# anibali/dsnt-pose2d

Measured on AMD Instinct MI355X. Metric: images/sec (train step, 256x256, 16 joints), higher is better.
Workload: dtype f32; 1 GPU; hg2 + DSNT + JS reg, 256x256 -> 64x64x16, batch 32 per GPU, RMSprop lr 2.5e-4, train step fwd+loss+bwd+optim; global_batch=32, parallelism=dp1, launches_fwd=210

## Files before the change

### dsnt-pose2d_amd/csrc/api.cpp

```cpp
#include "common.h"
#include <string.h>

static thread_local char g_err[512] = "";

int dsnt_set_error(int code, const char* fmt, ...) {
    va_list ap;
    va_start(ap, fmt);
    vsnprintf(g_err, sizeof(g_err), fmt, ap);
    va_end(ap);
    return code;
}

int dsnt_device_id(void) {
    int d = 0;
    if (hipGetDevice(&d) != hipSuccess || d < 0) d = 0;
    return d < DSNT_MAX_DEVICES ? d : DSNT_MAX_DEVICES - 1;
}

int dsnt_device_cus(void) {
    static std::atomic<int> cus[DSNT_MAX_DEVICES];
    const int d = dsnt_device_id();
    int c = cus[d].load(std::memory_order_acquire);
    if (!c) {
        hipDeviceProp_t prop;
        int dev = 0;
        c = (hipGetDevice(&dev) == hipSuccess && hipGetDeviceProperties(&prop, dev) == hipSuccess && prop.multiProcessorCount > 0)
                ? prop.multiProcessorCount : 256;
        cus[d].store(c, std::memory_order_release);
    }
    return c;
}

extern "C" int dsnt_version(void) { return 132; }
extern "C" const char* dsnt_last_error(void) { return g_err; }

#include <vector>
#include <new>

struct dsnt_list {
    struct Entry {
        int kind;
        int lane, src, dst;
        mutable hipEvent_t ev;
        std::function<void(hipStream_t)> fn;
    };
    std::vector<Entry> entries;
    std::vector<size_t> seg_start;
    dsnt_list() { seg_start.push_back(0); }
};

static thread_local dsnt_list* g_rec = nullptr;

dsnt_list* dsnt_recording(void) { return g_rec; }

void dsnt_record_launch(dsnt_list* l, int lane, std::function<void(hipStream_t)>&& fn) {
    dsnt_list::Entry e;
    e.kind = 0; e.lane = lane; e.src = e.dst = 0; e.ev = nullptr; e.fn = std::move(fn);
    l->entries.push_back(std::move(e));
}

extern "C" dsnt_list* dsnt_list_create(void) { return new (std::nothrow) dsnt_list(); }

extern "C" void dsnt_list_destroy(dsnt_list* l) {
    if (!l) return;
    if (g_rec == l) g_rec = nullptr;
    for (auto& e : l->entries)
// ... 60 lines not shown
```

### dsnt-pose2d_amd/csrc/bn.hip

```cpp
#include "common.h"
#include <string.h>
#include "bn_pro.h"
#include "ew_bodies.h"

template <int MODE>
__global__ __launch_bounds__(256) void tile_reduce_kernel(
    const float* __restrict__ a, const float* __restrict__ x, const float* __restrict__ scale,
    const float* __restrict__ shift, const float* __restrict__ mean,
    const float* __restrict__ invstd, int relu, float* __restrict__ partial, long M, int C, int cgs,
    const float* __restrict__ ymask = nullptr, float* __restrict__ dz_out = nullptr) {
    __shared__ float red[256 * 8];
    const int tid = threadIdx.x;
    const int C4 = C >> 2;
    const int rpar = 256 / cgs;
    const int cg_l = tid % cgs, rl = tid / cgs;
    const bool active = rl < rpar;
    const long row0 = (long)blockIdx.x * TILE_ROWS;
    const long row1 = row0 + TILE_ROWS < M ? row0 + TILE_ROWS : M;
    for (int cg0 = blockIdx.y * cgs; cg0 < C4; cg0 += cgs * gridDim.y) {
        const int cg = cg0 + cg_l;
        float4 s1 = make_float4(0.f, 0.f, 0.f, 0.f), s2 = s1;
        if (active && cg < C4) {
            float4 sc, sh, mu, is;
            if (MODE == 1) {
// ... 452 lines not shown

static int bn_bwd_pro_fill(BnBwdProP& q, const char* who, const float* partial, int ntiles, float* dgamma, float* dbeta,
                           int accumulate_params, float* coef, int64_t M, int C) {
    DSNT_REQUIRE(partial && ntiles > 0 && coef && C <= 256 && (long)ntiles * C <= 16384, DSNT_ERR_ARG,
                 "%s: needs partial sums of at most 256 channels / 128 KB and a coef buffer", who);
    q.partial = partial; q.tiles = ntiles; q.C = C; q.invM = 1.0 / (double)M;
    q.dgamma = dgamma; q.dbeta = dbeta; q.accumulate = accumulate_params; q.coef = coef;
    return DSNT_OK;
}

extern "C" int dsnt_bn_act_bwd_apply_pro(const float* da, const float* x, const float* scale, const float* shift,
                                         const float* mean, const float* invstd, const float* partial, int ntiles,
                                         float* dgamma, float* dbeta, int accumulate_params, float* coef, int relu,
                                         float* dx, int accumulate, int64_t M, int C, float* amax, void* stream) {
    BnBwdProP q;
    if (int e = bn_bwd_pro_fill(q, "dsnt_bn_act_bwd_apply_pro", partial, ntiles, dgamma, dbeta, accumulate_params, coef, M, C)) return e;
    return bn_act_bwd_apply_impl(da, x, scale, shift, mean, invstd, coef, relu, dx, accumulate, M, C, amax, stream, &q, nullptr);
}
extern "C" int dsnt_bn_act_bwd_apply_base(const float* da, const float* x, const float* scale, const float* shift,
                                          const float* mean, const float* invstd, const float* coef, int relu,
                                          const float* base, float* dx, int64_t M, int C, float* amax, void* stream) {
    DSNT_REQUIRE(base && base != dx, DSNT_ERR_ARG, "dsnt_bn_act_bwd_apply_base: `base` must be a second tensor");
    return bn_act_bwd_apply_impl(da, x, scale, shift, mean, invstd, coef, relu, dx, 1, M, C, amax, stream, nullptr, base);
}
extern "C" int dsnt_bn_act_bwd_apply_pro_base(const float* da, const float* x, const float* scale, const float* shift,
                                              const float* mean, const float* invstd, const float* partial, int ntiles,
                                              float* dgamma, float* dbeta, int accumulate_params, float* coef, int relu,
                                              const float* base, float* dx, int64_t M, int C, float* amax, void* stream) {
    DSNT_REQUIRE(base && base != dx, DSNT_ERR_ARG, "dsnt_bn_act_bwd_apply_pro_base: `base` must be a second tensor");
    BnBwdProP q;
    if (int e = bn_bwd_pro_fill(q, "dsnt_bn_act_bwd_apply_pro_base", partial, ntiles, dgamma, dbeta, accumulate_params, coef, M, C)) return e;
    return bn_act_bwd_apply_impl(da, x, scale, shift, mean, invstd, coef, relu, dx, 1, M, C, amax, stream, &q, base);
}
```

### dsnt-pose2d_amd/dsnt/_lib.py

```python
import ctypes as C
import os

import torch

_HERE = os.path.dirname(os.path.abspath(__file__))
LIB_PATH = os.environ.get('DSNT_HIP_LIB') or os.path.join(os.path.dirname(_HERE), 'csrc', 'libdsnt_hip.so')

P = C.c_void_p
I = C.c_int
L = C.c_int64
F = C.c_float
D = C.c_double


class ConvGeom(C.Structure):
    _fields_ = [(n, C.c_int) for n in
                ('N', 'H', 'W', 'Cin', 'Ho', 'Wo', 'Cout', 'R', 'S', 'stride', 'pad', 'dil')]


GP = C.POINTER(ConvGeom)


class BnBwdEpilogue(C.Structure):
    _fields_ = [('x', C.c_void_p), ('scale', C.c_void_p), ('shift', C.c_void_p), ('mean', C.c_void_p),
# ... 64 lines not shown
    'dsnt_conv_pack_dgrad': [P, P, I, I, I, I, P],
    'dsnt_conv_pack_dgrad_all': [P, I, P, P, P, L, P],
    'dsnt_conv_fwd_bf16x6': [P, P, L, P, P, P, P, I, P, P, P, GP, P],
    'dsnt_split_bf16x3': [P, P, L, P],
    'dsnt_conv_fwd_f16x3_ex': [P, P, L, P, P, P, P, P, P, I, P, P, P, GP, BP, TP, P],
    'dsnt_conv_fwd_f16x3_stream': [P, P, L, P, P, P, P, P, P, I, P, P, P, GP, BP, TP, P],
    'dsnt_amax': [P, L, P, P],
    'dsnt_split_f16x2': [P, P, L, L, P, P],
    'dsnt_f16_prep_weights': [P, I, I, P],
    'dsnt_f16_prep_bn_bounds': [P, I, P],
    'dsnt_conv_wgrad': [P, P, P, I, P, P, P, P, I, GP, P],
    'dsnt_conv_wgrad_bf16x6': [P, P, P, I, P, P, P, P, I, GP, P],
    'dsnt_conv_wgrad_f16x3': [P, P, P, I, P, P, P, P, I, P, P, GP, P],
    'dsnt_conv1x1_fwd_f16x3': [P, P, L, P, P, P, P, P, P, I, P, P, GP, TP, P],
    'dsnt_conv1x1_bwd_f16x3': [BP, P, AP, P, L, P, P, P, P, P, P, P, I, GP, P],
    'dsnt_conv1x1_fwd_ds_f16x3': [P, P, P, P, L, P, P, P, P, P, P, P, P, P, I, P, GP, GP, TP, P],
    'dsnt_conv_dgrad_f16x3_stream_apply': [P, AP, P, P, L, P, P, P, P, I, GP, BP, TP, P],
    'dsnt_wgrad_reduce_all': [P, I, I, P],
    'dsnt_conv_wgrad_group': [P, I, I, P],
    'dsnt_bn_stats': [P, P, L, I, P],
    'dsnt_bn_finalize': [P, I, L, I, P, P, P, P, F, F, I, P, P, P, P, P],
    'dsnt_bn_act_fwd': [P, P, P, I, P, L, I, P],
    'dsnt_bn_act_bwd_reduce': [P, P, P, P, P, P, I, P, L, I, P],
    'dsnt_bn_bwd_finalize': [P, I, L, I, P, P, I, P, P],
    'dsnt_bn_bwd_finalize_bound': [P, I, L, I, P, P, I, P, P, P, P, P],
    'dsnt_bn_eval_prep': [P, I, P],
    'dsnt_bn_act_bwd_apply': [P, P, P, P, P, P, P, I, P, I, L, I, P],
    'dsnt_bn_act_bwd_apply_amax': [P, P, P, P, P, P, P, I, P, I, L, I, P, P],
    'dsnt_bn_act_bwd_apply_pro': [P, P, P, P, P, P, P, I, P, P, I, P, I, P, I, L, I, P, P],
    'dsnt_stem4_fwd_f16x3': [P, P, L, P, P, P, P, P, GP, TP, P],
    'dsnt_bn_add_act_bwd_reduce': [P, P, P, P, P, I, P, P, L, I, P],
    'dsnt_bn_act_bwd_apply_base': [P, P, P, P, P, P, P, I, P, P, L, I, P, P],
    'dsnt_bn_act_bwd_apply_pro_base': [P, P, P, P, P, P, P, I, P, P, I, P, I, P, P, L, I, P, P],
    'dsnt_conv_fwd_pro': [P, P, P, P, PP, I, P, P, P, GP, TP, P],
    'dsnt_fill_zero': [P, L, P],
    'dsnt_axpy_amax': [P, P, F, I, L, P, P],
    'dsnt_maxpool2_bwd_amax': [P, P, P, I, I, I, I, I, P, P],
    'dsnt_maxpool2_bwd_add': [P, P, P, I, P, I, I, I, I, P, P],
    'dsnt_upsample2_bwd_amax': [P, P, I, I, I, I, I, P, P],
    'dsnt_maxpool2_fwd': [P, P, P, I, I, I, I, P],
    'dsnt_maxpool2_bwd': [P, P, P, I, I, I, I, I, P],
    'dsnt_maxpool2_fwd_stats': [P, P, P, P, I, I, I, I, TP, P],
    'dsnt_upsample2_add_fwd_stats': [P, P, P, P, I, I, I, I, TP, P],
    'dsnt_bn_act_fwd_stats': [P, P, P, I, P, P, L, I, TP, P],
    'dsnt_s2d_input': [P, P, I, I, I, I, TP, P],
    'dsnt_s2d_weights': [P, P, I, I, P],
    'dsnt_s2d_weights_prep': [P, P, P, P, P, I, P],
    'dsnt_maxpool3s2_fwd': [P, P, P, I, I, I, I, P],
    'dsnt_maxpool3s2_bwd': [P, P, P, I, I, I, I, I, P],
    'dsnt_bn_add_act_fwd': [P, P, P, P, I, P, L, I, P],
    'dsnt_relu_bwd': [P, P, P, L, P],
    'dsnt_zero_insert': [P, P, I, I, I, I, I, I, I, P],
    'dsnt_conv_dgrad_strided': [P, P, P, P, P, GP, BP, TP, P],
    'dsnt_upsample2_add_fwd': [P, P, P, I, I, I, I, P],
    'dsnt_upsample2_bwd': [P, P, I, I, I, I, I, P],
    'dsnt_axpy': [P, P, F, I, L, P],
    'dsnt_nchw_to_nhwc': [P, P, I, I, I, I, P],
    'dsnt_nhwc_to_nchw': [P, P, I, I, I, I, P],
    'dsnt_rmsprop_step': [P, P, P, L, F, F, F, F, F, P],
    'dsnt_sgd_step': [P, P, P, L, F, F, F, F, I, P],
    'dsnt_rmsprop_step_guarded': [P, P, P, L, F, F, F, F, F, P, P],
    'dsnt_sgd_step_guarded': [P, P, P, L, F, F, F, F, I, P, P],
    'dsnt_nonfinite_flag': [P, L, P, I, P],
    'dsnt_pckh': [P, P, P, P, P, P, F, P, P, I, I, P],
    'dsnt_pckh_hist': [P, P, P, P, P, P, P, I, P, P, I, I, P],
    'dsnt_error_field': [P, P, P, P, P, P, F, P, I, P, P, I, I, P],
# ... 113 lines not shown
```

### dsnt-pose2d_amd/dsnt/engine.py

```python
import os

import torch

from . import _lib, convop
from ._lib import ConvGeom, BnTail
from .bounds import Bounds
from .launchlist import Lanes, LaunchList
from .wgrad_queue import WgradQueue

BN_EPS = 1e-5
BN_MOMENTUM = 0.1


class Act:
    __slots__ = ('buf', 'N', 'H', 'W', 'C', '_grad', 'stats', 'name', 'grad_amax', 'amax_tail', 'fold_ok',
                 'pending_apply', 'uses', 'gives_away', 'is_branch', 'grad_shared', 'pending_add', 'base', 'base_amax')

    def __init__(self, buf, name=''):
        self.buf = buf
        self.N, self.H, self.W, self.C = buf.shape
        self._grad = None
        self.base, self.base_amax = None, None
        self.stats = None
        self.amax_tail = None
# ... 29 lines not shown
class ConvParams:
    __slots__ = ('w', 'b', 'gw', 'gb', 'Cout', 'R', 'S', 'Cin', 'stride', 'pad', 'dil', 'wq', 'wq_stride', 'wq16', 'wb',
                 'post_reduce')

    def __init__(self, w, b, gw, gb, stride=1, pad=0, dil=1):
        self.w, self.b, self.gw, self.gb = w, b, gw, gb
        self.wq, self.wq_stride = None, 0
        self.wq16, self.wb = None, None
        self.post_reduce = None
        self.Cout, self.R, self.S, self.Cin = w.shape
        self.stride, self.pad, self.dil = stride, pad, dil


class BnParams:
    __slots__ = ('gamma', 'beta', 'ggamma', 'gbeta', 'rmean', 'rvar', 'C', 'uses', 'momentum', 'eps')

    def __init__(self, gamma, beta, ggamma, gbeta, rmean, rvar, momentum=BN_MOMENTUM, eps=BN_EPS):
        self.gamma, self.beta, self.ggamma, self.gbeta = gamma, beta, ggamma, gbeta
        self.rmean, self.rvar = rmean, rvar
        self.momentum, self.eps = float(momentum), float(eps)
        self.C = gamma.numel()
        self.uses = 0


class Normed:
    __slots__ = ('x', 'bn', 'mean', 'invstd', 'scale', 'shift', 'relu', 'abound', 'pending', 'lane')


class PendingApply:
    __slots__ = ('dz', 'n', 'coef', 'bound', 'dz_amax')

    def __init__(self, dz, n, coef, bound, dz_amax):
        self.dz, self.n, self.coef, self.bound, self.dz_amax = dz, n, coef, bound, dz_amax


class Tape:
    def __init__(self, device, training, record=None, want_input_grad=False):
        self.device = device
        self.training = training
        self.record = training if record is None else bool(record)
        self.want_input_grad = want_input_grad
        self._bwd_emitters = []
        self._scratch = {}
        self._keep = []
        self.lib = _lib.load()
        self.nbytes = 0
        self._read_switches()
        lanes = Lanes(self.use_lanes, self.n_lanes)
        self.fwd, self.bwd = (LaunchList(self.lib, lanes, self._keep) for _ in range(2))
        self.bounds = Bounds(self)
        self.wgrads = WgradQueue(self)
        self.lane = 0
        self.cur_bucket = 0
        self._ident = None
        self.acts = []
        self.param_arena = None
        self._planar_src = {}
        self.f16_uses = []

    def _read_switches(self):
        self.use_bf16x6 = os.environ.get('DSNT_MFMA', 'bf16x6') != 'f32'
        self.bf16x6_min_rows = int(os.environ.get('DSNT_BF16X6_MIN_ROWS', '4096'))
        self.use_lanes = os.environ.get('DSNT_LANES', '1') != '0'
        self.side_lanes = (1, 3)
        self.n_lanes = 3 + len(self.side_lanes) - 1
        self.chain_lanes = (0,) + self.side_lanes
        self.wgrad_lane = 2 if (self.use_lanes and os.environ.get('DSNT_WGRAD_LANE', '1') != '0') else None
        self.wgrad_lane_rows = int(os.environ.get('DSNT_X_WGRAD_LANE_ROWS', '16000'))
        self.release_rows = int(os.environ.get('DSNT_X_RELEASE_ROWS', '4096'))
        off = set(os.environ.get('DSNT_OFF', '').replace('+', ',').split(','))
        self.conv3s = 'conv3s' not in off
        self.bwd1 = 'bwd1' not in off
        self.fwd1 = 'fwd1' not in off
        self.fold3 = 'fold3' not in off
        self.fold3_rows = int(os.environ.get('DSNT_X_FOLD3_ROWS', '16384'))
        self.stem4 = 'stem4' not in off
        self.ds_fuse = 'dsfuse' not in off
        self.ds_fuse_rows = int(os.environ.get('DSNT_X_DS_FUSE_ROWS', '65536'))
        self._x = dict(kv.split('=') for kv in os.environ.get('DSNT_X', '').split(',') if '=' in kv)
        self.wgrad_narrow = self._x.get('wgrad_narrow', '1')
        self.share_grads = self._x.get('share_grads', '1') != '0'
        self.defer_res = self._x.get('defer_res', '1') != '0'
        self.flush_points = self._x.get('flush_points', '1') != '0'
        self.prep_split = self._x.get('prep_split', '1') != '0'
        self.defer_reduce = os.environ.get('DSNT_DEFER_REDUCE', '1') != '0'
        self.group_rows = int(os.environ.get('DSNT_X_GROUP_ROWS', '8192')) if self.defer_reduce else 0
        self.fuse_finalize = os.environ.get('DSNT_FUSE_FINALIZE', '1') != '0'
        self.fuse_finalize_max = int(os.environ.get('DSNT_X_FUSE_FINALIZE_MAX', '2048'))
        self.use_f16x3 = self.use_bf16x6 and os.environ.get('DSNT_SPLIT', 'f16x3') == 'f16x3'
        if self.record and not self.training:
            self.use_f16x3 = False
        self.no_relu = bool(os.environ.get('DSNT_DEBUG_NO_RELU'))

    def empty(self, *shape, dtype=torch.float32):
        t = torch.empty(*shape, device=self.device, dtype=dtype)
        self.nbytes += t.numel() * t.element_size()
        self._keep.append(t)
        return t

    def scratch(self, key, numel, dtype=torch.float32, least=1):
        key = (key, self.lane)
        t = self._scratch.get(key)
        if t is None or t.numel() < numel:
            if t is not None:
                self._keep.append(t)
            t = torch.empty(max(numel, least), device=self.device, dtype=dtype)
            self.nbytes += t.numel() * t.element_size()
            self._scratch[key] = t
        return t

    def upload(self, rows, dtype=torch.int64):
        t = torch.tensor(rows, dtype=dtype).to(self.device)
# ... 168 lines not shown
        n.lane = self.lane
        if self.training:
            n.pending = self.ensure_stats(x)
            if not self.finalize_in_consumer(bn, n.pending[1]):
                self.materialize(n)
        else:
            self.bounds.eval_bn(n)
        return n

    def check_lane(self, n):
        if n.pending is not None:
            n.lane = self.lane
        elif n.lane != self.lane:
            raise RuntimeError('dsnt: BatchNorm vectors finalised on lane %d are read on lane %d without a synchronisation '
                               '(trace norm() and its consumers on one lane, or sync the lanes)' % (n.lane, self.lane))

    def materialize(self, n):
        self.check_lane(n)
        if n.pending is not None:
            part, tiles = n.pending
            n.pending = None
            bn = n.bn
            self.f('dsnt_bn_finalize', part, tiles, n.x.M, bn.C, bn.gamma, bn.beta, bn.rmean, bn.rvar,
                   bn.momentum, bn.eps, 1, n.mean, n.invstd, n.scale, n.shift)

    def fold_ok(self, n):
        x = n.x
        return bool(self.bwd1 and x.fold_ok and x.grad is None and x.pending_apply is None)

    def materialize_apply(self, x):
        ap, x.pending_apply = x.pending_apply, None
        n = ap.n
        buf, acc = self.grad_target(x, amax=True)
        self.b_amax('dsnt_bn_act_bwd_apply', ap.dz, x.buf, n.scale, n.shift, n.mean, n.invstd, ap.coef, 0,
                    buf, acc, x.M, n.bn.C, amax=x.grad_amax)

    def _norm_backward(self, n, da, reduced=None, finalised=False, dz_amax=None):
        x, bn = n.x, n.bn
        coef = self.scratch('bncoef', 2 * bn.C)
        relu = 1 if n.relu else 0
        if reduced is not None:
            part, tiles = reduced
            relu = 0
        else:
            tiles = (x.M + 127) // 128
            part = self.scratch('bnpart', tiles * 2 * bn.C).view(-1)
            self.b('dsnt_bn_act_bwd_reduce', da, x.buf, n.scale, n.shift, n.mean, n.invstd, relu, part,
                   x.M, bn.C)
        if dz_amax is not None:
            assert reduced is not None and not finalised and x.grad is None
            acc_p = 1 if bn.uses > 0 else 0
            bn.uses += 1
            coef = self.empty(2 * bn.C)
            bound = self.bounds.amax_slot()
            self.b('dsnt_bn_bwd_finalize_bound', part, tiles, x.M, bn.C, bn.ggamma, bn.gbeta, acc_p, coef, n.scale,
                   dz_amax, bound)
            x.pending_apply = PendingApply(da, n, coef, bound, dz_amax)
            return
        frozen = not self.training
        fused = (not finalised) and self.finalize_in_consumer(bn, tiles) and not frozen
        assert not (frozen and finalised)
        if not finalised:
            acc_p = 1 if bn.uses > 0 else 0
            bn.uses += 1
            if not fused:
                self.b('dsnt_bn_bwd_finalize', part, tiles, x.M, bn.C, bn.ggamma, bn.gbeta, acc_p | (2 if frozen else 0), coef)
        buf, acc, base = self.grad_target_base(x, amax=True)
        if fused:
            coef = self.empty(2 * bn.C)
            if base is not None:
                self.b('dsnt_bn_act_bwd_apply_pro_base', da, x.buf, n.scale, n.shift, n.mean, n.invstd, part, tiles,
                       bn.ggamma, bn.gbeta, acc_p, coef, relu, base, buf, x.M, bn.C, x.grad_amax)
            else:
                self.b('dsnt_bn_act_bwd_apply_pro', da, x.buf, n.scale, n.shift, n.mean, n.invstd, part, tiles,
                       bn.ggamma, bn.gbeta, acc_p, coef, relu, buf, acc, x.M, bn.C, x.grad_amax)
        elif base is not None:
            self.b('dsnt_bn_act_bwd_apply_base', da, x.buf, n.scale, n.shift, n.mean, n.invstd, coef, relu,
                   base, buf, x.M, bn.C, x.grad_amax)
        else:
            self.b_amax('dsnt_bn_act_bwd_apply', da, x.buf, n.scale, n.shift, n.mean, n.invstd, coef, relu,
                        buf, acc, x.M, bn.C, amax=x.grad_amax)

    def conv(self, src, p, res1=None, res2=None, want_stats=False, need_input_grad=True, name=''):
        c = convop.ConvOp(self, src, p, res1, res2, name, need_input_grad)
        c.y = y = self.act(c.x.N, c.g.Ho, c.g.Wo, p.Cout, name)
        c.x.uses += 1
        for r in (res1, res2):
            if r is not None:
                r.uses += 1
                y.gives_away = True
        c.forward(want_stats)
        if self.record:
            c.plan_backward()
            self.on_backward(c.backward)
        return y

    def ds_fuse_ok(self, x, p_ds, p3):
        return convop.ds_fuse_ok(self, x, p_ds, p3)

    def conv_ds(self, src, p, x_ds, p_ds, want_stats=False, name='', name_ds='ds'):
        c, cd = convop.ConvOp(self, src, p, None, None, name, True), convop.ConvOp(self, x_ds, p_ds, None, None, name_ds, True)
        c.y = cd.y = y = self.act(c.x.N, c.g.Ho, c.g.Wo, p.Cout, name)
        c.x.uses += 1
        x_ds.uses += 1
        c.forward_ds(cd, want_stats)
        cd.plan_backward()
        c.plan_backward()
        y.fold_ok = False
        self.on_backward(lambda: c.backward_ds(cd))
        return y

    def _f_with_stats(self, name, y, tensors, dims):
        part = None
        if self.training:
# ... 60 lines not shown
        self.f('dsnt_bn_add_act_fwd', x.buf, n.scale, n.shift, skip.buf, 1 if relu else 0, y.buf, x.M, x.C)
        if self.record:
            def backward():
                share = bool(self.share_grads and skip.untouched)
                if relu:
                    dz = (self.empty(x.M * x.C) if share else self.scratch('dz_tail', x.M * x.C).view(-1)[:x.M * x.C])
                    tiles = (x.M + 127) // 128
                    part = self.scratch('bnpart', tiles * 2 * bn.C).view(-1)
                    self.b('dsnt_bn_add_act_bwd_reduce', y.grad, y.buf, x.buf, n.mean, n.invstd, 1, dz, part, x.M, bn.C)
                    self._norm_backward(n, dz, reduced=(part, tiles))
                else:
                    dz = y.grad
                    self._norm_backward(n, dz)
                if share and skip.untouched:
                    skip.base, skip.base_amax = dz, None
                else:
                    self.grad_identity(skip, dz, donate=False)
            self.on_backward(backward)
        return y

    def upsample2_add(self, up, low, name=''):
        out = self.act(up.N, up.H, up.W, up.C, name)
        up.uses += 1
        low.uses += 1
        out.gives_away = True
        self._f_with_stats('dsnt_upsample2_add_fwd', out, (up.buf, low.buf, out.buf), (up.N, up.H, up.W, up.C))
        if self.record:
            point = self.wgrads.release_point(low.M)

            def backward():
                if point:
                    self.wgrads.pass_release_point()
                buf, acc = self.grad_target(low, amax=True)
                self.b_amax('dsnt_upsample2_bwd', out.grad, buf, acc, up.N, up.H, up.W, up.C, amax=low.grad_amax)
                self.grad_identity(up, out.grad, donate=True, g_amax=out.grad_amax)
            self.on_backward(backward)
        return out

    def to_planar(self, x, C_logical, name='', out=None, gin=None):
        out = self.empty(x.N, C_logical, x.H, x.W) if out is None else out
        x.uses += 1
        if gin is None:
            gin = self.empty(x.N, C_logical, x.H, x.W) if self.record else None
        self.f('dsnt_nhwc_to_nchw', x.buf, out, x.N, C_logical, x.H * x.W, x.C)
        if self.record:
            def backward():
                assert x.grad is None, 'planar output must be the first gradient writer'
                buf, _ = self.grad_target(x)
                self.b('dsnt_nchw_to_nhwc', gin, buf, x.N, C_logical, x.H * x.W, x.C)
            self.on_backward(backward)
        return out, gin

    def from_planar(self, src_nchw, Cpad, name=''):
        N, Cc, H, W = src_nchw.shape
        a = self.act(N, H, W, Cpad, name)
        e = self.f('dsnt_nchw_to_nhwc', src_nchw, a.buf, N, Cc, H * W, Cpad)
        self._planar_src[id(a)] = (src_nchw, e)
        return a

    def stem_s2d(self, x, p, name='stem'):
        got = self._planar_src.get(id(x))
        if (got is None or not self.use_f16x3 or p.R != 7 or p.S != 7 or p.stride != 2 or p.pad != 3
                or p.dil != 1 or x.C != 4 or x.H % 2 or x.W % 2 or x.N * (x.H // 2) * (x.W // 2) < self.bf16x6_min_rows):
            return None
        src, entry = got
        self.fwd.remove(entry)
        xs = self.act(x.N, x.H // 2 + 1, x.W // 2 + 1, 16, 'input_s2d')
# ... 15 lines not shown
```

### dsnt-pose2d_amd/dsnt/launchlist.py

```python
import contextlib
import ctypes as C

import torch

from . import _lib


def check(lib, rc, name):
    if rc != 0:
        raise RuntimeError('%s failed (%d): %s' % (name, rc, lib.dsnt_last_error().decode()))


class Lanes:

    def __init__(self, use, n):
        self.use, self.n = use, n
        self.side = None

    def streams(self):
        main = torch.cuda.current_stream()
        if not self.use:
            return (main, None, None)
        if self.side is None:
            self.side = tuple(torch.cuda.Stream() for _ in range(self.n - 1))
# ... 9 lines not shown
        self.nbytes, self.bytes_by_name = 0, {}
        self.workspace = set()
        self._into = self
        self._compiled = None

    @contextlib.contextmanager
    def into(self, lst):
        saved, self._into = self._into, lst
        try:
            yield lst
        finally:
            self._into = saved

    def count(self, name, nb):
        self.nbytes += nb
        self.bytes_by_name[name] = self.bytes_by_name.get(name, 0) + nb

    def emit(self, lane, name, *args):
        fn = getattr(self.lib, name)
        conv = []
        for a in args:
            if isinstance(a, torch.Tensor):
                if a.data_ptr() not in self.workspace:
                    self.count(name, a.numel() * a.element_size())
                conv.append(_lib.ptr(a))
            elif isinstance(a, C.Structure):
                self.keep.append(a)
                conv.append(C.byref(a))
            else:
                conv.append(a)
        entry = (fn, tuple(conv), name, lane)
        self._into.append(entry)
        return entry

    @staticmethod
    def sync_entry(src, dst):
        return (None, (src, dst, torch.cuda.Event()), 'sync', 0)

    def sync(self, src, dst):
        self._into.append(self.sync_entry(src, dst))

    def mark(self, k, lane):
        self._into.append((None, k, 'bucket', lane))

    def record(self):
        lib, lanes = self.lib, self.lanes
        h = lib.dsnt_list_create()
        if not h:
            raise RuntimeError('dsnt_list_create failed')
        marks = []
        try:
            for lane in range(1, lanes.n) if lanes.use else ():
                check(lib, lib.dsnt_list_sync(h, 0, lane), 'dsnt_list_sync')
            check(lib, lib.dsnt_list_begin(h), 'dsnt_list_begin')
            try:
                for fn, args, name, lane in self:
                    if fn is not None:
                        check(lib, fn(*args, C.c_void_p(lane)), name)
                    elif name == 'sync':
                        check(lib, lib.dsnt_list_sync(h, args[0], args[1]), 'dsnt_list_sync')
                    else:
                        marks.append((args, lane))
                        lib.dsnt_list_mark(h)
            finally:
                lib.dsnt_list_end()
            for lane in range(1, lanes.n) if lanes.use else ():
# ... 54 lines not shown
```

### include/dsnt_hip.h

```cpp
#ifndef DSNT_HIP_H
#define DSNT_HIP_H

#include <stdint.h>

#ifdef __cplusplus
extern "C" {
#endif

typedef enum {
    DSNT_OK = 0,
    DSNT_ERR_SHAPE = 1,
    DSNT_ERR_ALIGN = 2,
    DSNT_ERR_ARG = 3,
    DSNT_ERR_HIP = 4
} dsnt_status;

typedef struct {
    float* amax;
    float* amax_bn; const float* amax_scale; const float* amax_shift; int amax_relu, reserved;
} dsnt_out_bounds;

typedef struct dsnt_bn_prologue {
    const float* partial; int tiles, C;
    int64_t M;
// ... 221 lines not shown
                    float* y, int64_t M, int C, void* stream);

int dsnt_bn_eval_prep(const int64_t* table, int rows, void* stream);
#define DSNT_BN_FROZEN 2
int dsnt_bn_act_bwd_reduce(const float* da, const float* x, const float* scale,
                           const float* shift, const float* mean, const float* invstd,
                           int relu, float* partial, int64_t M, int C, void* stream);
int dsnt_bn_add_act_bwd_reduce(const float* da, const float* y, const float* x, const float* mean, const float* invstd,
                               int relu, float* dz, float* partial, int64_t M, int C, void* stream);
int dsnt_bn_bwd_finalize(const float* partial, int ntiles, int64_t M, int C,
                         float* dgamma, float* dbeta, int accumulate, float* coef,
                         void* stream);
int dsnt_bn_bwd_finalize_bound(const float* partial, int ntiles, int64_t M, int C, float* dgamma, float* dbeta,
                               int accumulate, float* coef, const float* scale, const float* dz_amax, float* bound_out,
                               void* stream);
int dsnt_bn_act_bwd_apply(const float* da, const float* x, const float* scale,
                          const float* shift, const float* mean, const float* invstd,
                          const float* coef, int relu, float* dx, int accumulate,
                          int64_t M, int C, void* stream);
int dsnt_bn_act_bwd_apply_amax(const float* da, const float* x, const float* scale, const float* shift,
                               const float* mean, const float* invstd, const float* coef, int relu, float* dx,
                               int accumulate, int64_t M, int C, float* amax, void* stream);
int dsnt_bn_act_bwd_apply_pro(const float* da, const float* x, const float* scale, const float* shift,
                              const float* mean, const float* invstd, const float* partial, int ntiles,
                              float* dgamma, float* dbeta, int accumulate_params, float* coef, int relu,
                              float* dx, int accumulate, int64_t M, int C, float* amax, void* stream);
int dsnt_bn_act_bwd_apply_base(const float* da, const float* x, const float* scale, const float* shift,
                               const float* mean, const float* invstd, const float* coef, int relu,
                               const float* base, float* dx, int64_t M, int C, float* amax, void* stream);
int dsnt_bn_act_bwd_apply_pro_base(const float* da, const float* x, const float* scale, const float* shift,
                                   const float* mean, const float* invstd, const float* partial, int ntiles,
                                   float* dgamma, float* dbeta, int accumulate_params, float* coef, int relu,
                                   const float* base, float* dx, int64_t M, int C, float* amax, void* stream);
int dsnt_fill_zero(float* p, int64_t n, void* stream);
int dsnt_axpy_amax(const float* x, float* y, float a, int accumulate, int64_t n, float* amax, void* stream);
int dsnt_maxpool2_bwd_amax(const float* dy, const uint8_t* idx, float* dx, int accumulate, int N, int H, int W, int C,
                           float* amax, void* stream);
int dsnt_maxpool2_bwd_add(const float* dy, const uint8_t* idx, float* dx, int accumulate, const float* extra,
                          int N, int H, int W, int C, float* amax, void* stream);
int dsnt_upsample2_bwd_amax(const float* dout, float* dlow, int accumulate, int N, int H, int W, int C, float* amax,
                            void* stream);

int dsnt_maxpool2_fwd(const float* x, float* y, uint8_t* idx, int N, int H, int W, int C,
                      void* stream);
int dsnt_maxpool2_bwd(const float* dy, const uint8_t* idx, float* dx, int accumulate,
                      int N, int H, int W, int C, void* stream);

int dsnt_maxpool3s2_fwd(const float* x, float* y, uint8_t* idx, int N, int H, int W, int C, void* stream);
int dsnt_maxpool3s2_bwd(const float* dy, const uint8_t* idx, float* dx, int accumulate, int N, int H, int W,
                        int C, void* stream);
int dsnt_bn_add_act_fwd(const float* x, const float* scale, const float* shift, const float* res, int relu,
                        float* y, int64_t M, int C, void* stream);
int dsnt_relu_bwd(const float* dy, const float* y, float* dz, int64_t n, void* stream);
int dsnt_zero_insert(const float* dy, float* out, int N, int Ho, int Wo, int C, int Hs, int Ws, int stride,
                     void* stream);

int dsnt_conv_dgrad_strided(const float* dy, const float* wd, float* dx, const float* res1, float* stats_partial,
                            const dsnt_conv_geom* g, const dsnt_bn_bwd_epilogue* bnb, const dsnt_out_bounds* tail, void* stream);
int dsnt_conv_dgrad_strided_ok(const dsnt_conv_geom* g);
int dsnt_conv_dgrad_strided_tiles(const dsnt_conv_geom* g);

int dsnt_upsample2_add_fwd(const float* up, const float* low, float* out,
                           int N, int H, int W, int C, void* stream);
int dsnt_upsample2_bwd(const float* dout, float* dlow, int accumulate,
                       int N, int H, int W, int C, void* stream);

// ... 164 lines not shown
```

Before: 2941 images/sec.

## Fuse BN backward apply with following upsample-backward or BN reduce

Adds two fused kernels. One does the BN-activation backward apply and also the 2x upsample backward, writing dx and the pooled low-resolution gradient in the same pass. The other does the apply and also the next BN's backward reduction, so it emits per-tile partial sums. A tape-level peephole finds the most recent apply that produced the source gradient and rewrites that launch in place. This saves re-reading the large gradient tensor and one launch per fused pair, but adds more complex dependency checks in the launch list.

```diff
diff --git a/dsnt-pose2d_amd/csrc/api.cpp b/dsnt-pose2d_amd/csrc/api.cpp
--- a/dsnt-pose2d_amd/csrc/api.cpp
+++ b/dsnt-pose2d_amd/csrc/api.cpp
@@ -31,7 +31,7 @@
     return c;
 }
 
-extern "C" int dsnt_version(void) { return 132; }
+extern "C" int dsnt_version(void) { return 133; }
 extern "C" const char* dsnt_last_error(void) { return g_err; }
 
 #include <vector>
diff --git a/dsnt-pose2d_amd/csrc/bn.hip b/dsnt-pose2d_amd/csrc/bn.hip
--- a/dsnt-pose2d_amd/csrc/bn.hip
+++ b/dsnt-pose2d_amd/csrc/bn.hip
@@ -508,3 +508,193 @@
     if (int e = bn_bwd_pro_fill(q, "dsnt_bn_act_bwd_apply_pro_base", partial, ntiles, dgamma, dbeta, accumulate_params, coef, M, C)) return e;
     return bn_act_bwd_apply_impl(da, x, scale, shift, mean, invstd, coef, relu, dx, 1, M, C, amax, stream, &q, base);
 }
+
+__device__ __forceinline__ float4 bn_apply_dx(const float4 g, const float4 xv, const BnApplyVec& v, int relu, bool accumulate, const float4 p) {
+    float4 o = bn_apply_one(g, xv, v, relu);
+    {
+#pragma clang fp contract(off)
+        if (accumulate) { o.x += p.x; o.y += p.y; o.z += p.z; o.w += p.w; }
+    }
+    return o;
+}
+
+struct BnApplyUpP { BnApplyP a; float4* dlow; int accumulate_low; int N, H, W; unsigned* amax_low; };
+template <bool FIXED>
+__global__ __launch_bounds__(256) void bn_act_bwd_apply_up_kernel(BnApplyUpP q) {
+    const float4* __restrict__ da = q.a.da; const float4* __restrict__ x = q.a.x; const float4* __restrict__ scale = q.a.scale;
+    const float4* __restrict__ shift = q.a.shift; const float4* __restrict__ mean = q.a.mean; const float4* __restrict__ invstd = q.a.invstd;
+    const float4* __restrict__ coef = q.a.coef; const int relu = q.a.relu; float4* dx = q.a.dx; const float4* base = q.a.base;
+    const int C4 = q.a.C4; unsigned* amax = q.a.amax; float4* dlow = q.dlow; const int accumulate_low = q.accumulate_low;
+    const int N = q.N, H = q.H, W = q.W; unsigned* amax_low = q.amax_low;
+    const bool accumulate = base != nullptr;
+    const int Hl = H >> 1, Wl = W >> 1;
+    const long total = (long)N * Hl * Wl * C4;
+    const long stride = (long)gridDim.x * 256;
+    float am = 0.f, aml = 0.f;
+    auto vec = [&](int cg) {
+        BnApplyVec v;
+        v.sc = scale[cg]; v.sh = shift[cg]; v.mu = mean[cg]; v.is = invstd[cg]; v.c0 = coef[cg]; v.c1 = coef[C4 + cg];
+        return v;
+    };
+    long i = (long)blockIdx.x * 256 + threadIdx.x;
+    BnApplyVec vf;
+    if (FIXED) vf = vec((int)((i < total ? i : 0) % C4));
+    for (; i < total; i += stride) {
+        const int cg = (int)(i % C4);
+        long t = i / C4;
+        const int w = (int)(t % Wl); t /= Wl;
+        const int h = (int)(t % Hl);
+        const int n = (int)(t / Hl);
+        const long b = (((long)n * H + 2 * h) * W + 2 * w) * C4 + cg;
+        const long off[4] = {b, b + C4, b + (long)W * C4, b + (long)W * C4 + C4};
+        float4 g[4], xv[4], p[4];
+#pragma unroll
+        for (int k = 0; k < 4; ++k) { g[k] = da[off[k]]; xv[k] = x[off[k]]; }
+#pragma unroll
+        for (int k = 0; k < 4; ++k) p[k] = accumulate ? base[off[k]] : make_float4(0.f, 0.f, 0.f, 0.f);
+        const BnApplyVec v = FIXED ? vf : vec(cg);
+        float4 o[4];
+#pragma unroll
+        for (int k = 0; k < 4; ++k) {
+            o[k] = bn_apply_dx(g[k], xv[k], v, relu, accumulate, p[k]);
+            dx[off[k]] = o[k];
+            am = fmaxf(fmaxf(fmaxf(fabsf(o[k].x), fabsf(o[k].y)), fmaxf(fabsf(o[k].z), fabsf(o[k].w))), am);
+        }
+        {
+#pragma clang fp contract(off)
+            float4 l = make_float4((o[0].x + o[1].x) + (o[2].x + o[3].x), (o[0].y + o[1].y) + (o[2].y + o[3].y),
+                                   (o[0].z + o[1].z) + (o[2].z + o[3].z), (o[0].w + o[1].w) + (o[2].w + o[3].w));
+            if (accumulate_low) { const float4 c = dlow[i]; l.x += c.x; l.y += c.y; l.z += c.z; l.w += c.w; }
+            dlow[i] = l;
+            aml = fmaxf(fmaxf(fmaxf(fabsf(l.x), fabsf(l.y)), fmaxf(fabsf(l.z), fabsf(l.w))), aml);
+        }
+    }
+    if (amax) amax_commit(am, amax, 0);
+    if (amax_low) amax_commit(aml, amax_low, 1);
+}
+
+extern "C" int dsnt_bn_act_bwd_apply_up(const float* da, const float* x, const float* scale, const float* shift,
+                                        const float* mean, const float* invstd, const float* coef, int relu,
+                                        const float* base, float* dx, int64_t M, int C, float* amax, int N, int H, int W,
+                                        float* dlow, int accumulate_low, float* amax_low, void* stream) {
+    DSNT_REQUIRE(da && x && scale && shift && mean && invstd && coef && dx && dlow && M > 0 && C > 0 && N > 0 && H > 0 && W > 0,
+                 DSNT_ERR_ARG, "dsnt_bn_act_bwd_apply_up: bad argument");
+    DSNT_REQUIRE(H % 2 == 0 && W % 2 == 0 && (int64_t)N * H * W == M, DSNT_ERR_SHAPE,
+                 "dsnt_bn_act_bwd_apply_up: H and W must be even and N*H*W == M");
+    DSNT_REQUIRE(C % 4 == 0 && dsnt_aligned16(da) && dsnt_aligned16(x) && dsnt_aligned16(dx) && dsnt_aligned16(coef) &&
+                 dsnt_aligned16(base) && dsnt_aligned16(dlow) && dsnt_aligned16(scale) && dsnt_aligned16(shift) &&
+                 dsnt_aligned16(mean) && dsnt_aligned16(invstd), DSNT_ERR_ALIGN, "dsnt_bn_act_bwd_apply_up: alignment");
+    DSNT_REQUIRE(dlow != dx && (const float*)dlow != base && (const float*)dlow != da, DSNT_ERR_ARG,
+                 "dsnt_bn_act_bwd_apply_up: `dlow` must be a tensor of its own");
+    const long total = (long)N * (H / 2) * (W / 2) * (C / 4);
+    const int grid = flat_grid(total, 256);
+    BnBwdProP nopro;
+    memset(&nopro, 0, sizeof(nopro));
+    const BnApplyUpP q{BnApplyP{(const float4*)da, (const float4*)x, (const float4*)scale, (const float4*)shift, (const float4*)mean,
+                                (const float4*)invstd, (const float4*)coef, relu, (float4*)dx, (const float4*)base, (long)M * C / 4,
+                                C / 4, (unsigned*)amax, nopro},
+                       (float4*)dlow, accumulate_low, N, H, W, (unsigned*)amax_low};
+    if (((long)grid * 256) % (C / 4) == 0)
+        DSNT_LAUNCH(bn_act_bwd_apply_up_kernel<true>, dim3(grid), dim3(256), 0, stream, q);
+    else
+        DSNT_LAUNCH(bn_act_bwd_apply_up_kernel<false>, dim3(grid), dim3(256), 0, stream, q);
+    DSNT_CHECK_LAUNCH("dsnt_bn_act_bwd_apply_up");
+}
+
+struct BnApplyRedP {
+    BnApplyP a; const float* x2; const float* scale2; const float* shift2; const float* mean2; const float* invstd2; int relu2;
+    float* partial; long M; int C, cgs;
+};
+__global__ __launch_bounds__(256) void bn_act_bwd_apply_reduce_kernel(BnApplyRedP q) {
+    __shared__ float red[256 * 8];
+    const float4* __restrict__ da = q.a.da; const float4* __restrict__ xa = q.a.x; const int relu_a = q.a.relu;
+    float4* dx = q.a.dx; const float4* base = q.a.base; unsigned* amax = q.a.amax;
+    const float* __restrict__ x = q.x2; const float* __restrict__ scale = q.scale2; const float* __restrict__ shift = q.shift2;
+    const float* __restrict__ mean = q.mean2; const float* __restrict__ invstd = q.invstd2; const int relu = q.relu2;
+    float* __restrict__ partial = q.partial; const long M = q.M; const int C = q.C, cgs = q.cgs;
+    const bool accumulate = base != nullptr;
+    const int tid = threadIdx.x;
+    const int C4 = C >> 2;
+    const int rpar = 256 / cgs;
+    const int cg_l = tid % cgs, rl = tid / cgs;
+    const bool active = rl < rpar;
+    const long row0 = (long)blockIdx.x * TILE_ROWS;
+    const long row1 = row0 + TILE_ROWS < M ? row0 + TILE_ROWS : M;
+    float am = 0.f;
+    for (int cg0 = blockIdx.y * cgs; cg0 < C4; cg0 += cgs * gridDim.y) {
+        const int cg = cg0 + cg_l;
+        float4 s1 = make_float4(0.f, 0.f, 0.f, 0.f), s2 = s1;
+        if (active && cg < C4) {
+            BnApplyVec v;
+            v.sc = q.a.scale[cg]; v.sh = q.a.shift[cg]; v.mu = q.a.mean[cg]; v.is = q.a.invstd[cg];
+            v.c0 = q.a.coef[cg]; v.c1 = q.a.coef[C4 + cg];
+            const float4 sc = reinterpret_cast<const float4*>(scale)[cg];
+            const float4 sh = reinterpret_cast<const float4*>(shift)[cg];
+            const float4 mu = reinterpret_cast<const float4*>(mean)[cg];
+            const float4 is = reinterpret_cast<const float4*>(invstd)[cg];
+            for (long r = row0 + rl; r < row1; r += rpar) {
+                const long e = r * C4 + cg;
+                const float4 g = da[e], xg = xa[e];
+                const float4 xv = reinterpret_cast<const float4*>(x + r * C)[cg];
+                const float4 p = accumulate ? base[e] : make_float4(0.f, 0.f, 0.f, 0.f);
+                const float4 o = bn_apply_dx(g, xg, v, relu_a, accumulate, p);
+                dx[e] = o;
+                am = fmaxf(fmaxf(fmaxf(fabsf(o.x), fabsf(o.y)), fmaxf(fabsf(o.z), fabsf(o.w))), am);
+                {
+#pragma clang fp contract(off)
+                    float4 dz = o;
+                    if (relu) {
+                        if (fmaf(xv.x, sc.x, sh.x) <= 0.f) dz.x = 0.f;
+                        if (fmaf(xv.y, sc.y, sh.y) <= 0.f) dz.y = 0.f;
+                        if (fmaf(xv.z, sc.z, sh.z) <= 0.f) dz.z = 0.f;
+                        if (fmaf(xv.w, sc.w, sh.w) <= 0.f) dz.w = 0.f;
+                    }
+                    s1.x += dz.x; s1.y += dz.y; s1.z += dz.z; s1.w += dz.w;
+                    s2.x = fmaf(dz.x, (xv.x - mu.x) * is.x, s2.x);
+                    s2.y = fmaf(dz.y, (xv.y - mu.y) * is.y, s2.y);
+                    s2.z = fmaf(dz.z, (xv.z - mu.z) * is.z, s2.z);
+                    s2.w = fmaf(dz.w, (xv.w - mu.w) * is.w, s2.w);
+                }
+            }
+        }
+        __syncthreads();
+        float* mine = red + tid * 8;
+        mine[0] = s1.x; mine[1] = s1.y; mine[2] = s1.z; mine[3] = s1.w;
+        mine[4] = s2.x; mine[5] = s2.y; mine[6] = s2.z; mine[7] = s2.w;
+        __syncthreads();
+        if (tid < cgs && cg0 + tid < C4) {
+            float acc[8] = {0, 0, 0, 0, 0, 0, 0, 0};
+            for (int j = 0; j < rpar; ++j)
+#pragma unroll
+                for (int e = 0; e < 8; ++e) acc[e] += red[(j * cgs + tid) * 8 + e];
+            float* p0 = partial + ((size_t)blockIdx.x * 2 + 0) * C + (size_t)(cg0 + tid) * 4;
+            float* p1 = partial + ((size_t)blockIdx.x * 2 + 1) * C + (size_t)(cg0 + tid) * 4;
+            *reinterpret_cast<float4*>(p0) = make_float4(acc[0], acc[1], acc[2], acc[3]);
+            *reinterpret_cast<float4*>(p1) = make_float4(acc[4], acc[5], acc[6], acc[7]);
+        }
+    }
+    if (amax) amax_commit(am, amax);
+}
+
+extern "C" int dsnt_bn_act_bwd_apply_reduce(const float* da, const float* x, const float* scale, const float* shift,
+                                            const float* mean, const float* invstd, const float* coef, int relu, float* dx,
+                                            int accumulate, const float* x2, const float* scale2, const float* shift2,
+                                            const float* mean2, const float* invstd2, int relu2, float* partial, int64_t M, int C,
+                                            float* amax, void* stream) {
+    DSNT_REQUIRE(da && x && scale && shift && mean && invstd && coef && dx && x2 && scale2 && shift2 && mean2 && invstd2 &&
+                 partial && M > 0 && C > 0, DSNT_ERR_ARG, "dsnt_bn_act_bwd_apply_reduce: bad argument");
+    DSNT_REQUIRE(C % 4 == 0 && dsnt_aligned16(da) && dsnt_aligned16(x) && dsnt_aligned16(dx) && dsnt_aligned16(coef) &&
+                 dsnt_aligned16(scale) && dsnt_aligned16(shift) && dsnt_aligned16(mean) && dsnt_aligned16(invstd) &&
+                 dsnt_aligned16(x2) && dsnt_aligned16(scale2) && dsnt_aligned16(shift2) && dsnt_aligned16(mean2) &&
+                 dsnt_aligned16(invstd2) && dsnt_aligned16(partial), DSNT_ERR_ALIGN,
+                 "dsnt_bn_act_bwd_apply_reduce: C %% 4 and 16-byte alignment required");
+    const int tiles = (int)((M + TILE_ROWS - 1) / TILE_ROWS);
+    BnBwdProP nopro;
+    memset(&nopro, 0, sizeof(nopro));
+    const BnApplyRedP q{BnApplyP{(const float4*)da, (const float4*)x, (const float4*)scale, (const float4*)shift, (const float4*)mean,
+                                 (const float4*)invstd, (const float4*)coef, relu, (float4*)dx, accumulate ? (const float4*)dx : nullptr,
+                                 (long)M * C / 4, C / 4, (unsigned*)amax, nopro},
+                        x2, scale2, shift2, mean2, invstd2, relu2, partial, (long)M, C, tile_cgs(tiles, C / 4)};
+    DSNT_LAUNCH(bn_act_bwd_apply_reduce_kernel, dim3(tiles, tile_grid_y(tiles, C / 4)), dim3(256), 0, stream, q);
+    DSNT_CHECK_LAUNCH("dsnt_bn_act_bwd_apply_reduce");
+}
diff --git a/dsnt-pose2d_amd/dsnt/_lib.py b/dsnt-pose2d_amd/dsnt/_lib.py
--- a/dsnt-pose2d_amd/dsnt/_lib.py
+++ b/dsnt-pose2d_amd/dsnt/_lib.py
@@ -120,6 +120,8 @@
     'dsnt_bn_add_act_bwd_reduce': [P, P, P, P, P, I, P, P, L, I, P],
     'dsnt_bn_act_bwd_apply_base': [P, P, P, P, P, P, P, I, P, P, L, I, P, P],
     'dsnt_bn_act_bwd_apply_pro_base': [P, P, P, P, P, P, P, I, P, P, I, P, I, P, P, L, I, P, P],
+    'dsnt_bn_act_bwd_apply_up': [P, P, P, P, P, P, P, I, P, P, L, I, P, I, I, I, P, I, P, P],
+    'dsnt_bn_act_bwd_apply_reduce': [P, P, P, P, P, P, P, I, P, I, P, P, P, P, P, I, P, L, I, P, P],
     'dsnt_conv_fwd_pro': [P, P, P, P, PP, I, P, P, P, GP, TP, P],
     'dsnt_fill_zero': [P, L, P],
     'dsnt_axpy_amax': [P, P, F, I, L, P, P],
diff --git a/dsnt-pose2d_amd/dsnt/engine.py b/dsnt-pose2d_amd/dsnt/engine.py
--- a/dsnt-pose2d_amd/dsnt/engine.py
+++ b/dsnt-pose2d_amd/dsnt/engine.py
@@ -85,6 +85,17 @@
 
     def __init__(self, dz, n, coef, bound, dz_amax):
         self.dz, self.n, self.coef, self.bound, self.dz_amax = dz, n, coef, bound, dz_amax
+
+
+class ApplyLaunch:
+    __slots__ = ('entry', 'vecs', 'base', 'buf', 'acc', 'M', 'C', 'amax')
+
+    def __init__(self, entry, vecs, base, buf, acc, M, C, amax):
+        self.entry, self.vecs, self.base, self.buf, self.acc, self.M, self.C, self.amax = entry, vecs, base, buf, acc, M, C, amax
+
+    @property
+    def tensors(self):
+        return self.vecs + (self.base, self.buf, self.amax)
 
 
 class Tape:
@@ -110,6 +121,7 @@
         self.param_arena = None
         self._planar_src = {}
         self.f16_uses = []
+        self._applies = {}
 
     def _read_switches(self):
         self.use_bf16x6 = os.environ.get('DSNT_MFMA', 'bf16x6') != 'f32'
@@ -131,6 +143,9 @@
         self.ds_fuse = 'dsfuse' not in off
         self.ds_fuse_rows = int(os.environ.get('DSNT_X_DS_FUSE_ROWS', '65536'))
         self._x = dict(kv.split('=') for kv in os.environ.get('DSNT_X', '').split(',') if '=' in kv)
+        self.apply_up = 'applyup' not in off
+        self.apply_red = 'applyred' not in off
+        self.apply_fuse_rows = int(self._x.get('APPLY_FUSE_ROWS', os.environ.get('DSNT_X_APPLY_FUSE_ROWS', '32768')))
         self.wgrad_narrow = self._x.get('wgrad_narrow', '1')
         self.share_grads = self._x.get('share_grads', '1') != '0'
         self.defer_res = self._x.get('defer_res', '1') != '0'
@@ -365,8 +380,7 @@
         ap, x.pending_apply = x.pending_apply, None
         n = ap.n
         buf, acc = self.grad_target(x, amax=True)
-        self.b_amax('dsnt_bn_act_bwd_apply', ap.dz, x.buf, n.scale, n.shift, n.mean, n.invstd, ap.coef, 0,
-                    buf, acc, x.M, n.bn.C, amax=x.grad_amax)
+        self._emit_apply(ap.dz, x, n, ap.coef, 0, None, buf, acc)
 
     def _norm_backward(self, n, da, reduced=None, finalised=False, dz_amax=None):
         x, bn = n.x, n.bn
@@ -378,8 +392,9 @@
         else:
             tiles = (x.M + 127) // 128
             part = self.scratch('bnpart', tiles * 2 * bn.C).view(-1)
-            self.b('dsnt_bn_act_bwd_reduce', da, x.buf, n.scale, n.shift, n.mean, n.invstd, relu, part,
-                   x.M, bn.C)
+            if not self._fuse_apply_reduce(da, n, relu, part):
+                self.b('dsnt_bn_act_bwd_reduce', da, x.buf, n.scale, n.shift, n.mean, n.invstd, relu, part,
+                       x.M, bn.C)
         if dz_amax is not None:
             assert reduced is not None and not finalised and x.grad is None
             acc_p = 1 if bn.uses > 0 else 0
@@ -407,12 +422,58 @@
             else:
                 self.b('dsnt_bn_act_bwd_apply_pro', da, x.buf, n.scale, n.shift, n.mean, n.invstd, part, tiles,
                        bn.ggamma, bn.gbeta, acc_p, coef, relu, buf, acc, x.M, bn.C, x.grad_amax)
-        elif base is not None:
-            self.b('dsnt_bn_act_bwd_apply_base', da, x.buf, n.scale, n.shift, n.mean, n.invstd, coef, relu,
-                   base, buf, x.M, bn.C, x.grad_amax)
         else:
-            self.b_amax('dsnt_bn_act_bwd_apply', da, x.buf, n.scale, n.shift, n.mean, n.invstd, coef, relu,
-                        buf, acc, x.M, bn.C, amax=x.grad_amax)
+            self._emit_apply(da, x, n, coef, relu, base, buf, acc)
+
+    def _emit_apply(self, da, x, n, coef, relu, base, buf, acc):
+        vecs = (da, x.buf, n.scale, n.shift, n.mean, n.invstd, coef, relu)
+        if base is not None:
+            e = self.b('dsnt_bn_act_bwd_apply_base', *vecs, base, buf, x.M, n.bn.C, x.grad_amax)
+        else:
+            e = self.b_amax('dsnt_bn_act_bwd_apply', *vecs, buf, acc, x.M, n.bn.C, amax=x.grad_amax)
+        self._applies[id(e)] = ApplyLaunch(e, vecs, base, buf, acc, x.M, n.bn.C, x.grad_amax)
+
+    def _fusable_apply(self, src, written):
+        lst = self.bwd
+        if lst._into is not lst:
+            return None
+        sp, wp = src.data_ptr(), [t.data_ptr() for t in written]
+        for i in range(len(lst) - 1, -1, -1):
+            e = lst[i]
+            if e[0] is None:
+                if e[2] != 'sync' or e[1][1] == self.lane:
+                    return None
+            elif lst.names(e, sp):
+                ap = self._applies.get(id(e))
+                if ap is None or ap.entry is not e or e[3] != self.lane or ap.buf.data_ptr() != sp or ap.M < self.apply_fuse_rows:
+                    return None
+                return i, ap
+            elif e[2] in ('dsnt_conv_wgrad_group', 'dsnt_wgrad_reduce_all') or any(lst.names(e, p) for p in wp):
+                return None
+        return None
+
+    def _fuse_apply_up(self, out_grad, up, dlow, acc_low, amax_low):
+        got = self._fusable_apply(out_grad, [dlow]) if self.apply_up else None
+        if got is None or got[1].M != up.M or got[1].C != up.C:
+            return False
+        i, ap = got
+        base = ap.base if ap.base is not None else (ap.buf if ap.acc else None)
+        self.bwd.replace(i, ap.tensors, self.lane, 'dsnt_bn_act_bwd_apply_up', *ap.vecs, base, ap.buf, ap.M, ap.C, ap.amax,
+                         up.N, up.H, up.W, dlow, acc_low, amax_low)
+        if base is ap.buf:
+            self.bwd.count('dsnt_bn_act_bwd_apply_up', -base.numel() * base.element_size())
+        del self._applies[id(ap.entry)]
+        return True
+
+    def _fuse_apply_reduce(self, da, n, relu, part):
+        got = self._fusable_apply(da, [part]) if self.apply_red else None
+        if got is None or got[1].base is not None or got[1].M != n.x.M or got[1].C != n.bn.C:
+            return False
+        i, ap = got
+        self.bwd.replace(i, ap.tensors, self.lane, 'dsnt_bn_act_bwd_apply_reduce', *ap.vecs, ap.buf, ap.acc, n.x.buf, n.scale,
+                         n.shift, n.mean, n.invstd, relu, part, ap.M, ap.C, ap.amax)
+        del self._applies[id(ap.entry)]
+        return True
 
     def conv(self, src, p, res1=None, res2=None, want_stats=False, need_input_grad=True, name=''):
         c = convop.ConvOp(self, src, p, res1, res2, name, need_input_grad)
@@ -539,7 +600,8 @@
                 if point:
                     self.wgrads.pass_release_point()
                 buf, acc = self.grad_target(low, amax=True)
-                self.b_amax('dsnt_upsample2_bwd', out.grad, buf, acc, up.N, up.H, up.W, up.C, amax=low.grad_amax)
+                if not self._fuse_apply_up(out.grad, up, buf, acc, low.grad_amax):
+                    self.b_amax('dsnt_upsample2_bwd', out.grad, buf, acc, up.N, up.H, up.W, up.C, amax=low.grad_amax)
                 self.grad_identity(up, out.grad, donate=True, g_amax=out.grad_amax)
             self.on_backward(backward)
         return out
diff --git a/dsnt-pose2d_amd/dsnt/launchlist.py b/dsnt-pose2d_amd/dsnt/launchlist.py
--- a/dsnt-pose2d_amd/dsnt/launchlist.py
+++ b/dsnt-pose2d_amd/dsnt/launchlist.py
@@ -65,6 +65,19 @@
         entry = (fn, tuple(conv), name, lane)
         self._into.append(entry)
         return entry
+
+    def replace(self, i, old_args, lane, name, *args):
+        old = self[i][2]
+        for a in old_args:
+            if isinstance(a, torch.Tensor) and a.data_ptr() not in self.workspace:
+                self.count(old, -a.numel() * a.element_size())
+        with self.into([]):
+            self[i] = self.emit(lane, name, *args)
+        return self[i]
+
+    @staticmethod
+    def names(entry, ptr):
+        return any(getattr(a, 'value', a) == ptr for a in entry[1] if isinstance(a, (int, C.c_void_p)))
 
     @staticmethod
     def sync_entry(src, dst):
diff --git a/include/dsnt_hip.h b/include/dsnt_hip.h
--- a/include/dsnt_hip.h
+++ b/include/dsnt_hip.h
@@ -277,6 +277,15 @@
                                    const float* mean, const float* invstd, const float* partial, int ntiles,
                                    float* dgamma, float* dbeta, int accumulate_params, float* coef, int relu,
                                    const float* base, float* dx, int64_t M, int C, float* amax, void* stream);
+int dsnt_bn_act_bwd_apply_up(const float* da, const float* x, const float* scale, const float* shift,
+                             const float* mean, const float* invstd, const float* coef, int relu,
+                             const float* base, float* dx, int64_t M, int C, float* amax, int N, int H, int W,
+                             float* dlow, int accumulate_low, float* amax_low, void* stream);
+int dsnt_bn_act_bwd_apply_reduce(const float* da, const float* x, const float* scale, const float* shift,
+                                 const float* mean, const float* invstd, const float* coef, int relu, float* dx,
+                                 int accumulate, const float* x2, const float* scale2, const float* shift2,
+                                 const float* mean2, const float* invstd2, int relu2, float* partial, int64_t M, int C,
+                                 float* amax, void* stream);
 int dsnt_fill_zero(float* p, int64_t n, void* stream);
 int dsnt_axpy_amax(const float* x, float* y, float a, int accumulate, int64_t n, float* amax, void* stream);
 int dsnt_maxpool2_bwd_amax(const float* dy, const uint8_t* idx, float* dx, int accumulate, int N, int H, int W, int C,
```

Result: no change. 2957 images/sec, median of 6 (+0.5%).
